# exfinen/zk-toolkit

Hardware: AMD Instinct MI355X
Metric: G1 MSM scalar-muls/sec at 2^20 bases per GPU (BLS12-381) (higher is better)
Workload: dtype u32 limbs (384-bit Montgomery integer)

## Files before the change

zk-toolkit_amd/csrc/curve.h:

```cpp
#pragma once
#include "tower.h"

namespace zkt {

template <class C> struct PrimeOps {
  typedef Fp<C> E;
  ZKT_HD static E zero() { return fp_zero<C>(); }
  ZKT_HD static E one() { return fp_one<C>(); }
  ZKT_HD static E add(const E& a, const E& b) { return fp_add(a, b); }
  ZKT_HD static E sub(const E& a, const E& b) { return fp_sub(a, b); }
  ZKT_HD static E mul(const E& a, const E& b) { return fp_mul(a, b); }
  ZKT_HD static E sqr(const E& a) { return fp_sqr(a); }
  ZKT_HD static E dbl(const E& a) { return fp_dbl(a); }
  ZKT_HD static E sub2(const E& a, const E& b, const E& c) { return fp_sub2(a, b, c); }
  ZKT_HD static E mulsub(const E& a, const E& b, const E& c, const E& d) { return fp_mulsub(a, b, c, d); }
  ZKT_HD static E neg(const E& a) { return fp_neg(a); }
  ZKT_HD static E inv(const E& a) { return fp_inv(a); }
  ZKT_HD static bool is_zero(const E& a) { return fp_is_zero(a); }
  ZKT_HD static bool eq(const E& a, const E& b) { return fp_eq(a, b); }
};
typedef PrimeOps<FqC> FqOps;
typedef PrimeOps<SpC> SpOps;
struct Fq2Ops {
  typedef Fq2 E;
  ZKT_HD static E zero() { return fq2_zero(); }
  ZKT_HD static E one() { return fq2_one(); }
  ZKT_HD static E add(const E& a, const E& b) { return fq2_add(a, b); }
  ZKT_HD static E sub(const E& a, const E& b) { return fq2_sub(a, b); }
  ZKT_HD static E mul(const E& a, const E& b) { return fq2_mul(a, b); }
  ZKT_HD static E sqr(const E& a) { return fq2_sqr(a); }
  ZKT_HD static E dbl(const E& a) { return fq2_dbl(a); }
  ZKT_HD static E sub2(const E& a, const E& b, const E& c) { return fq2_sub2(a, b, c); }
  ZKT_HD static E mulsub(const E& a, const E& b, const E& c, const E& d) { return fq2_mulsub(a, b, c, d); }
  ZKT_HD static E neg(const E& a) { return fq2_neg(a); }
  ZKT_HD static E inv(const E& a) { return fq2_inv(a); }
  ZKT_HD static bool is_zero(const E& a) { return fq2_is_zero(a); }
  ZKT_HD static bool eq(const E& a, const E& b) { return fq2_eq(a, b); }
};

template <class F> struct Aff { typename F::E x, y; bool inf; };
template <class F> struct Jac { typename F::E X, Y, Z; };
template <class F> struct Xyzz { typename F::E X, Y, ZZ, ZZZ; };

template <class F> ZKT_HD Jac<F> jac_inf() { return Jac<F>{F::one(), F::one(), F::zero()}; }
template <class F> ZKT_HD bool jac_is_inf(const Jac<F>& p) { return F::is_zero(p.Z); }
template <class F> ZKT_HD Jac<F> jac_from_aff(const Aff<F>& a) {
  if (a.inf) return jac_inf<F>();
  return Jac<F>{a.x, a.y, F::one()};
}

template <class F> ZKT_HD Jac<F> jac_dbl(const Jac<F>& p) {
  typedef typename F::E E;
  E A = F::sqr(p.X), B = F::sqr(p.Y), C = F::sqr(B);
  E t = F::sqr(F::add(p.X, B));
  E D = F::dbl(F::sub(F::sub(t, A), C));
  E Ee = F::add(F::dbl(A), A);
  E Ff = F::sqr(Ee);
  Jac<F> r;
  r.X = F::sub2(Ff, F::zero(), D);
  E C8 = F::dbl(F::dbl(F::dbl(C)));
  r.Y = F::sub(F::mul(Ee, F::sub(D, r.X)), C8);
  r.Z = F::dbl(F::mul(p.Y, p.Z));
  return r;
}

template <class F> ZKT_HD Jac<F> jac_add_aff(const Jac<F>& p, const Aff<F>& q) {
  typedef typename F::E E;
  if (q.inf) return p;
  if (jac_is_inf(p)) return Jac<F>{q.x, q.y, F::one()};
  E ZZ = F::sqr(p.Z);
  E U2 = F::mul(q.x, ZZ);
  E S2 = F::mul(F::mul(q.y, p.Z), ZZ);
  E H = F::sub(U2, p.X);
  E Rr = F::sub(S2, p.Y);
  if (F::is_zero(H)) {
    if (F::is_zero(Rr)) return jac_dbl(Jac<F>{q.x, q.y, F::one()});
    return jac_inf<F>();
  }
  E HH = F::sqr(H), HHH = F::mul(H, HH), V = F::mul(p.X, HH);
  Jac<F> r;
  r.X = F::sub2(F::sqr(Rr), HHH, V);
  r.Y = F::mulsub(Rr, F::sub(V, r.X), p.Y, HHH);
  r.Z = F::mul(p.Z, H);
  return r;
}

template <class F> ZKT_HD Jac<F> jac_add(const Jac<F>& p, const Jac<F>& q) {
  typedef typename F::E E;
  if (jac_is_inf(q)) return p;
  if (jac_is_inf(p)) return q;
  E Z1Z1 = F::sqr(p.Z), Z2Z2 = F::sqr(q.Z);
  E U1 = F::mul(p.X, Z2Z2), U2 = F::mul(q.X, Z1Z1);
  E S1 = F::mul(F::mul(p.Y, q.Z), Z2Z2), S2 = F::mul(F::mul(q.Y, p.Z), Z1Z1);
  E H = F::sub(U2, U1), Rr = F::sub(S2, S1);
  if (F::is_zero(H)) {
    if (F::is_zero(Rr)) return jac_dbl(p);
    return jac_inf<F>();
  }
  E HH = F::sqr(H), HHH = F::mul(H, HH), V = F::mul(U1, HH);
  Jac<F> r;
  r.X = F::sub2(F::sqr(Rr), HHH, V);
  r.Y = F::mulsub(Rr, F::sub(V, r.X), S1, HHH);
  r.Z = F::mul(F::mul(p.Z, q.Z), H);
  return r;
}

template <class F> ZKT_HD Aff<F> jac_to_aff(const Jac<F>& p) {
  typedef typename F::E E;
  Aff<F> a;
  if (jac_is_inf(p)) { a.x = F::zero(); a.y = F::zero(); a.inf = true; return a; }
  E zi = F::inv(p.Z), zi2 = F::sqr(zi);
  a.x = F::mul(p.X, zi2);
  a.y = F::mul(p.Y, F::mul(zi2, zi));
  a.inf = false;
  return a;
}

template <class F> ZKT_HD Xyzz<F> xyzz_inf() { return Xyzz<F>{F::one(), F::one(), F::zero(), F::zero()}; }
template <class F> ZKT_HD bool xyzz_is_inf(const Xyzz<F>& p) { return F::is_zero(p.ZZ); }
template <class F> ZKT_HD Xyzz<F> xyzz_dbl_aff(const typename F::E& x, const typename F::E& y) {
  typedef typename F::E E;
  if (F::is_zero(y)) return xyzz_inf<F>();
  E U = F::dbl(y), V = F::sqr(U), W = F::mul(U, V), S = F::mul(x, V);
  E xx = F::sqr(x), M = F::add(F::dbl(xx), xx);
  Xyzz<F> r;
  r.X = F::sub2(F::sqr(M), F::zero(), S);
  r.Y = F::mulsub(M, F::sub(S, r.X), W, y);
  r.ZZ = V; r.ZZZ = W;
  return r;
}
template <class F> ZKT_HD Xyzz<F> xyzz_dbl(const Xyzz<F>& p) {
  typedef typename F::E E;
  if (xyzz_is_inf(p) || F::is_zero(p.Y)) return xyzz_inf<F>();
  E U = F::dbl(p.Y), V = F::sqr(U), W = F::mul(U, V), S = F::mul(p.X, V);
  E xx = F::sqr(p.X), M = F::add(F::dbl(xx), xx);
  Xyzz<F> r;
  r.X = F::sub2(F::sqr(M), F::zero(), S);
  r.Y = F::mulsub(M, F::sub(S, r.X), W, p.Y);
  r.ZZ = F::mul(V, p.ZZ); r.ZZZ = F::mul(W, p.ZZZ);
  return r;
}
template <class F> ZKT_HD Xyzz<F> xyzz_add_aff(const Xyzz<F>& p, const typename F::E& x2, const typename F::E& y2) {
  typedef typename F::E E;
  if (xyzz_is_inf(p)) return Xyzz<F>{x2, y2, F::one(), F::one()};
  E U2 = F::mul(x2, p.ZZ), S2 = F::mul(y2, p.ZZZ);
  E Pp = F::sub(U2, p.X), Rr = F::sub(S2, p.Y);
  if (F::is_zero(Pp)) {
    if (F::is_zero(Rr)) return xyzz_dbl_aff<F>(x2, y2);
    return xyzz_inf<F>();
  }
  E PP = F::sqr(Pp), PPP = F::mul(Pp, PP), Qq = F::mul(p.X, PP);
  Xyzz<F> r;
  r.X = F::sub2(F::sqr(Rr), PPP, Qq);
  r.Y = F::mulsub(Rr, F::sub(Qq, r.X), p.Y, PPP);
  r.ZZ = F::mul(p.ZZ, PP); r.ZZZ = F::mul(p.ZZZ, PPP);
  return r;
}
template <class F> ZKT_HD Xyzz<F> xyzz_add(const Xyzz<F>& p, const Xyzz<F>& q) {
  typedef typename F::E E;
  if (xyzz_is_inf(q)) return p;
  if (xyzz_is_inf(p)) return q;
  E U1 = F::mul(p.X, q.ZZ), U2 = F::mul(q.X, p.ZZ);
  E S1 = F::mul(p.Y, q.ZZZ), S2 = F::mul(q.Y, p.ZZZ);
  E Pp = F::sub(U2, U1), Rr = F::sub(S2, S1);
  if (F::is_zero(Pp)) {
    if (F::is_zero(Rr)) return xyzz_dbl(p);
    return xyzz_inf<F>();
  }
  E PP = F::sqr(Pp), PPP = F::mul(Pp, PP), Qq = F::mul(U1, PP);
  Xyzz<F> r;
  r.X = F::sub2(F::sqr(Rr), PPP, Qq);
  r.Y = F::mulsub(Rr, F::sub(Qq, r.X), S1, PPP);
  r.ZZ = F::mul(F::mul(p.ZZ, q.ZZ), PP); r.ZZZ = F::mul(F::mul(p.ZZZ, q.ZZZ), PPP);
  return r;
}
template <class F> ZKT_HD Aff<F> xyzz_to_aff(const Xyzz<F>& p) {
  typedef typename F::E E;
  Aff<F> a;
  if (xyzz_is_inf(p)) { a.x = F::zero(); a.y = F::zero(); a.inf = true; return a; }
  E zi3 = F::inv(p.ZZZ);
  E zi2 = F::sqr(F::mul(zi3, p.ZZ));
  a.x = F::mul(p.X, zi2);
  a.y = F::mul(p.Y, zi3);
  a.inf = false;
  return a;
}
template <class F> ZKT_HD Jac<F> xyzz_to_jac(const Xyzz<F>& p) {
  if (xyzz_is_inf(p)) return jac_inf<F>();
  return Jac<F>{F::mul(p.X, p.ZZ), F::mul(p.Y, p.ZZZ), p.ZZ};
}

static constexpr int SCALAR_MAX_LIMBS = 12;
template <class F> ZKT_HD Jac<F> scalar_mul_aff(const Aff<F>& p, const uint32_t* k, int nlimbs) {
  Jac<F> acc = jac_inf<F>();
  if (p.inf) return acc;
  uint32_t nz[SCALAR_MAX_LIMBS + 1], ng[SCALAR_MAX_LIMBS + 1];
  uint32_t carry = 0;
  for (int w = 0; w <= nlimbs; ++w) {
    const uint32_t cur = w < nlimbs ? k[w] : 0u, nxt = w + 1 < nlimbs ? k[w + 1] : 0u;
    uint32_t znz = 0, zng = 0;
    for (int b = 0; b < 32; ++b) {
      const uint32_t b0 = (cur >> b) & 1, b1 = b < 31 ? (cur >> (b + 1)) & 1 : nxt & 1;
      const uint32_t x0 = b0 ^ carry;
      const uint32_t sum1 = b1 ^ (b0 & carry);
      const uint32_t neg = x0 & sum1;
      znz |= x0 << b; zng |= neg << b;
      carry = (b0 & carry) | (neg);
    }
    nz[w] = znz; ng[w] = zng;
  }
  Aff<F> q = p; q.y = F::neg(p.y);
  bool started = false;
  for (int i = nlimbs * 32; i >= 0; --i) {
    if (started) acc = jac_dbl(acc);
    if ((nz[i >> 5] >> (i & 31)) & 1) { acc = jac_add_aff(acc, ((ng[i >> 5] >> (i & 31)) & 1) ? q : p); started = true; }
  }
  return acc;
}

}
```

zk-toolkit_amd/csrc/fp.h:

```cpp
#pragma once
#include <stdint.h>
#include <hip/hip_runtime.h>
#include "zkt_constants.h"

namespace zkt {

template <class C>
struct Fp {
  typedef uint32_t vec_t __attribute__((ext_vector_type(C::N)));
  vec_t v;
};

ZKT_HD void mac(uint64_t& lo, uint32_t& hi, uint32_t a, uint32_t b) {
#if defined(__HIP_DEVICE_COMPILE__)
  asm("v_mad_u64_u32 %0, vcc, %2, %3, %0\n\tv_addc_co_u32 %1, vcc, 0, %1, vcc" : "+v"(lo), "+v"(hi) : "v"(a), "v"(b) : "vcc");
#else
  uint64_t p = (uint64_t)a * b; lo += p; hi += (lo < p);
#endif
}
ZKT_HD void mac_k(uint64_t& lo, uint32_t& hi, uint32_t a, uint32_t b) {
#if defined(__HIP_DEVICE_COMPILE__)
  asm("v_mad_u64_u32 %0, vcc, %2, %3, %0\n\tv_addc_co_u32 %1, vcc, 0, %1, vcc" : "+v"(lo), "+v"(hi) : "v"(a), "s"(b) : "vcc");
#else
  mac(lo, hi, a, b);
#endif
}
ZKT_HD uint32_t addc(uint32_t a, uint32_t b, uint32_t& c) { unsigned co; uint32_t r = __builtin_addc(a, b, c, &co); c = co; return r; }
ZKT_HD uint32_t subb(uint32_t a, uint32_t b, uint32_t& c) { unsigned co; uint32_t r = __builtin_subc(a, b, c, &co); c = co; return r; }

#define ZKT_FORCE_FRAME() do { alignas(64) volatile uint32_t zkt_frame_anchor_[16]; zkt_frame_anchor_[0] = 0u; } while (0)

template <class C> ZKT_HD Fp<C> fp_zero() { Fp<C> r;
#pragma unroll
  for (int i = 0; i < C::N; ++i) r.v[i] = 0; return r; }
template <class C> ZKT_HD Fp<C> fp_one() { Fp<C> r;
#pragma unroll
  for (int i = 0; i < C::N; ++i) r.v[i] = C::one(i); return r; }
template <class C> ZKT_HD bool fp_is_zero(const Fp<C>& a) {
  if constexpr (C::W == 28) {
    const uint32_t a0 = a.v[0];
    if (!((a0 == C::kp(0, 0)) | (a0 == C::kp(1, 0)) | (a0 == C::kp(2, 0)) | (a0 == C::kp(3, 0)))) return false;
    uint32_t o0 = 0, o1 = 0, o2 = 0, o3 = 0;
#pragma unroll
    for (int i = 0; i < C::N; ++i) { o0 |= a.v[i]; o1 |= a.v[i] ^ C::kp(1, i); o2 |= a.v[i] ^ C::kp(2, i); o3 |= a.v[i] ^ C::kp(3, i); }
    return (o0 == 0) | (o1 == 0) | (o2 == 0) | (o3 == 0);
  } else {
    uint32_t o = 0;
#pragma unroll
    for (int i = 0; i < C::N; ++i) o |= a.v[i];
    return o == 0;
  }
}

template <class C> ZKT_HD void fp_cond_sub(Fp<C>& r, uint32_t top) {
  uint32_t s[C::N]; uint32_t bw = 0;
#pragma unroll
  for (int i = 0; i < C::N; ++i) s[i] = subb(r.v[i], C::mod(i), bw);
  bool keep = (top == 0) && bw;
#pragma unroll
  for (int i = 0; i < C::N; ++i) r.v[i] = keep ? r.v[i] : s[i];
}

template <class C> ZKT_HD Fp<C> fp_lazy_reduce(const uint32_t* v) {
  constexpr uint32_t M = (1u << C::W) - 1;
  Fp<C> r; const uint32_t q = (uint32_t)(((uint64_t)v[C::N - 1] * C::QEST_M) >> 32);
  uint32_t carry = 0;
#pragma unroll
  for (int i = 0; i < C::N; ++i) {
    uint64_t t = (uint64_t)q * C::comp(i) + (uint64_t)(v[i] + carry);
    r.v[i] = (uint32_t)t & M; carry = (uint32_t)(t >> C::W);
  }
  return r;
}

template <class C> ZKT_HD Fp<C> fp_add(const Fp<C>& a, const Fp<C>& b) {
  if constexpr (C::W == 28) {
    uint32_t v[C::N];
#pragma unroll
    for (int i = 0; i < C::N; ++i) v[i] = a.v[i] + b.v[i];
    return fp_lazy_reduce<C>(v);
  } else {
    Fp<C> r; uint32_t c = 0;
#pragma unroll
    for (int i = 0; i < C::N; ++i) r.v[i] = addc(a.v[i], b.v[i], c);
    fp_cond_sub(r, c);
    return r;
  }
}
template <class C> ZKT_HD Fp<C> fp_sub(const Fp<C>& a, const Fp<C>& b) {
  if constexpr (C::W == 28) {
    uint32_t v[C::N];
#pragma unroll
    for (int i = 0; i < C::N; ++i) v[i] = a.v[i] + C::subk(i) - b.v[i];
    return fp_lazy_reduce<C>(v);
  } else {
    Fp<C> r; uint32_t bw = 0;
#pragma unroll
    for (int i = 0; i < C::N; ++i) r.v[i] = subb(a.v[i], b.v[i], bw);
    uint32_t mask = 0u - bw, c = 0;
#pragma unroll
    for (int i = 0; i < C::N; ++i) r.v[i] = addc(r.v[i], C::mod(i) & mask, c);
    return r;
  }
}
template <class C> ZKT_HD Fp<C> fp_neg(const Fp<C>& a) {
  if constexpr (C::W == 28) {
    return fp_sub(fp_zero<C>(), a);
  } else {
    Fp<C> r; uint32_t bw = 0;
#pragma unroll
    for (int i = 0; i < C::N; ++i) r.v[i] = subb(C::mod(i), a.v[i], bw);
    uint32_t mask = fp_is_zero(a) ? 0u : 0xffffffffu;
#pragma unroll
    for (int i = 0; i < C::N; ++i) r.v[i] &= mask;
    return r;
  }
}
template <class C> ZKT_HD bool fp_eq(const Fp<C>& a, const Fp<C>& b) {
  if constexpr (C::W == 28) {
    return fp_is_zero(fp_sub(a, b));
  } else {
    uint32_t o = 0;
#pragma unroll
    for (int i = 0; i < C::N; ++i) o |= a.v[i] ^ b.v[i];
    return o == 0;
  }
}
template <class C> ZKT_HD Fp<C> fp_dbl(const Fp<C>& a) { return fp_add(a, a); }
template <class C> ZKT_HD Fp<C> fp_add3(const Fp<C>& a, const Fp<C>& b, const Fp<C>& c) {
  if constexpr (C::W == 28) {
    uint32_t v[C::N];
#pragma unroll
    for (int i = 0; i < C::N; ++i) v[i] = a.v[i] + b.v[i] + c.v[i];
    return fp_lazy_reduce<C>(v);
  } else return fp_add(fp_add(a, b), c);
}
// ... 74 lines not shown
      lo = (lo >> 32) | ((uint64_t)hi << 32); hi = 0;
    }
    fp_cond_sub(r, (uint32_t)lo);
    return r;
  }
}

template <class C> ZKT_HD Fp<C> fp_sqr_impl(const Fp<C>& a) {
  static_assert(C::W == 28, "lazy-limb fields only");
  constexpr int N = C::N; constexpr uint32_t M = (1u << 28) - 1;
  Fp<C> r; uint32_t m[N], d[N]; uint64_t acc = 0;
#pragma unroll
  for (int i = 0; i < N; ++i) d[i] = a.v[i] << 1;
#pragma unroll
  for (int k = 0; k < 2 * N; ++k) {
#pragma unroll
    for (int i = (k < N ? 0 : k - N + 1); 2 * i < k; ++i) acc = mad64(d[i], a.v[k - i], acc);
    if ((k & 1) == 0) acc = mad64(a.v[k / 2], a.v[k / 2], acc);
    if (k < N) {
#pragma unroll
      for (int j = 0; j < k; ++j) acc = mad64(m[j], C::mod(k - j), acc);
      m[k] = ((uint32_t)acc * C::INV) & M;
      acc = mad64(m[k], C::mod(0), acc);
    } else {
#pragma unroll
      for (int j = k - N + 1; j < N; ++j) acc = mad64(m[j], C::mod(k - j), acc);
      r.v[k - N] = (uint32_t)acc & M;
    }
    acc >>= 28;
  }
  return r;
}

template <class C, bool SUB> ZKT_HD Fp<C> fp_mul2_impl(const Fp<C>& a, const Fp<C>& b, const Fp<C>& c, const Fp<C>& d) {
  static_assert(C::W == 28, "lazy-limb fields only");
  constexpr int N = C::N; constexpr uint32_t M = (1u << 28) - 1;
  Fp<C> r; uint32_t m[N], nd[N]; uint64_t acc = 0;
#pragma unroll
  for (int i = 0; i < N; ++i) nd[i] = SUB ? C::subk(i) - d.v[i] : d.v[i];
#pragma unroll
  for (int k = 0; k < 2 * N; ++k) {
#pragma unroll
    for (int i = (k < N ? 0 : k - N + 1); i <= (k < N ? k : N - 1); ++i) { acc = mad64(a.v[i], b.v[k - i], acc); acc = mad64(c.v[i], nd[k - i], acc); }
    if (k < N) {
#pragma unroll
      for (int j = 0; j < k; ++j) acc = mad64(m[j], C::mod(k - j), acc);
      m[k] = ((uint32_t)acc * C::INV) & M;
      acc = mad64(m[k], C::mod(0), acc);
    } else {
#pragma unroll
      for (int j = k - N + 1; j < N; ++j) acc = mad64(m[j], C::mod(k - j), acc);
      r.v[k - N] = (uint32_t)acc & M;
    }
    acc >>= 28;
  }
  return r;
}

template <class C> ZKT_HD void fp2_mul_kara(const Fp<C>& a0, const Fp<C>& a1, const Fp<C>& b0, const Fp<C>& b1, Fp<C>& re, Fp<C>& im) {
  static_assert(C::W == 28, "lazy-limb fields only");
  constexpr int N = C::N; constexpr uint32_t M = (1u << 28) - 1;
  uint32_t sa[N], sb[N], nd[N], mr[N], mi[N]; uint64_t accr = 0, acci = 0;
#pragma unroll
  for (int i = 0; i < N; ++i) { sa[i] = a0.v[i] + a1.v[i]; sb[i] = b0.v[i] + b1.v[i]; nd[i] = C::subk(i) - b1.v[i]; }
#pragma unroll
  for (int k = 0; k < 2 * N; ++k) {
    uint64_t p0 = 0, p1 = 0;
#pragma unroll
    for (int i = (k < N ? 0 : k - N + 1); i <= (k < N ? k : N - 1); ++i) {
      p0 = mad64(a0.v[i], b0.v[k - i], p0); p1 = mad64(a1.v[i], nd[k - i], p1); acci = mad64(sa[i], sb[k - i], acci);
    }
    accr += p0 + p1; acci += p1 - p0;
    if (k < N) {
#pragma unroll
      for (int j = 0; j < k; ++j) { accr = mad64(mr[j], C::mod(k - j), accr); acci = mad64(mi[j], C::mod(k - j), acci); }
      mr[k] = ((uint32_t)accr * C::INV) & M; mi[k] = ((uint32_t)acci * C::INV) & M;
      accr = mad64(mr[k], C::mod(0), accr); acci = mad64(mi[k], C::mod(0), acci);
    } else {
#pragma unroll
      for (int j = k - N + 1; j < N; ++j) { accr = mad64(mr[j], C::mod(k - j), accr); acci = mad64(mi[j], C::mod(k - j), acci); }
      re.v[k - N] = (uint32_t)accr & M; im.v[k - N] = (uint32_t)acci & M;
    }
    accr >>= 28; acci >>= 28;
  }
}

#if !defined(ZKT_INLINE_MUL)
template <class C> ZKT_FN Fp<C> fp_mul(Fp<C> a, Fp<C> b) { return fp_mul_impl(a, b); }
template <class C> ZKT_FN Fp<C> fp_sqr_fn(Fp<C> a) { return fp_sqr_impl(a); }
#if defined(ZKT_INLINE_MUL2)
template <class C> ZKT_HD Fp<C> fp_mulsub_fn(const Fp<C>& a, const Fp<C>& b, const Fp<C>& c, const Fp<C>& d) { return fp_mul2_impl<C, true>(a, b, c, d); }
template <class C> ZKT_HD Fp<C> fp_muladd_fn(const Fp<C>& a, const Fp<C>& b, const Fp<C>& c, const Fp<C>& d) { return fp_mul2_impl<C, false>(a, b, c, d); }
#else
template <class C> ZKT_FN Fp<C> fp_mulsub_fn(Fp<C> a, Fp<C> b, Fp<C> c, Fp<C> d) { return fp_mul2_impl<C, true>(a, b, c, d); }
template <class C> ZKT_FN Fp<C> fp_muladd_fn(Fp<C> a, Fp<C> b, Fp<C> c, Fp<C> d) { return fp_mul2_impl<C, false>(a, b, c, d); }
#endif
#else
template <class C> ZKT_HD Fp<C> fp_mul(const Fp<C>& a, const Fp<C>& b) { return fp_mul_impl(a, b); }
template <class C> ZKT_HD Fp<C> fp_sqr_fn(const Fp<C>& a) { return fp_sqr_impl(a); }
template <class C> ZKT_HD Fp<C> fp_mulsub_fn(const Fp<C>& a, const Fp<C>& b, const Fp<C>& c, const Fp<C>& d) { return fp_mul2_impl<C, true>(a, b, c, d); }
template <class C> ZKT_HD Fp<C> fp_muladd_fn(const Fp<C>& a, const Fp<C>& b, const Fp<C>& c, const Fp<C>& d) { return fp_mul2_impl<C, false>(a, b, c, d); }
#endif
template <class C> ZKT_HD Fp<C> fp_mulsub(const Fp<C>& a, const Fp<C>& b, const Fp<C>& c, const Fp<C>& d) {
  if constexpr (C::W == 28) return fp_mulsub_fn(a, b, c, d); else return fp_sub(fp_mul(a, b), fp_mul(c, d));
}
template <class C> ZKT_HD Fp<C> fp_muladd(const Fp<C>& a, const Fp<C>& b, const Fp<C>& c, const Fp<C>& d) {
  if constexpr (C::W == 28) return fp_muladd_fn(a, b, c, d); else return fp_add(fp_mul(a, b), fp_mul(c, d));
}

template <class C> ZKT_HD Fp<C> fp_sqr(const Fp<C>& a) {
  if constexpr (C::W == 28) return fp_sqr_fn(a); else return fp_mul(a, a);
}

template <class C> ZKT_HD Fp<C> fp_from_words(const uint32_t* w) {
  Fp<C> x, r2;
#pragma unroll
  for (int i = 0; i < C::N; ++i) r2.v[i] = C::r2(i);
  if constexpr (C::W == 28) {
#pragma unroll
    for (int i = 0; i < C::N; ++i) {
      const int lo = (28 * i) >> 5, sh = (28 * i) & 31;
      uint32_t t = w[lo] >> sh;
      if (sh > 4 && lo + 1 < C::ABI_N) t |= w[lo + 1] << (32 - sh);
      x.v[i] = t & 0x0fffffffu;
    }
  } else {
#pragma unroll
    for (int i = 0; i < C::N; ++i) x.v[i] = w[i];
    x = fp_canon32(x);
  }
  return fp_mul(x, r2);
}
template <class C> ZKT_HD void fp_to_words(const Fp<C>& a, uint32_t* w) {
  Fp<C> one = fp_zero<C>(); one.v[0] = 1;
  Fp<C> x = fp_mul(a, one);
  if constexpr (C::W == 28) {
    uint32_t s[C::N], bw = 0;
#pragma unroll
    for (int i = 0; i < C::N; ++i) { uint32_t t = x.v[i] - C::mod(i) - bw; bw = t >> 31; s[i] = t & 0x0fffffffu; }
#pragma unroll
    for (int i = 0; i < C::N; ++i) s[i] = bw ? x.v[i] : s[i];
#pragma unroll
    for (int j = 0; j < C::ABI_N; ++j) {
      uint32_t t = 0;
#pragma unroll
      for (int i = 0; i < C::N; ++i) {
        const int sft = 28 * i - 32 * j;
        if (sft > -28 && sft < 32) t |= sft >= 0 ? (s[i] << (sft & 31)) : (s[i] >> ((-sft) & 31));
      }
      w[j] = t;
    }
  } else {
#pragma unroll
    for (int i = 0; i < C::N; ++i) w[i] = x.v[i];
  }
}
template <class C> ZKT_HD Fp<C> fp_canon32(Fp<C> x) {
  static_assert(C::W == 32, "canonical 32-bit-limb fields only");
  fp_cond_sub(x, 0); fp_cond_sub(x, 0);
  return x;
}

template <class C> ZKT_HD void bgcd_inverse_classic(uint32_t* io) {
  constexpr int N = C::ABI_N;
  uint32_t u[N + 1], v[N + 1], x1[N + 1], x2[N + 1];
#pragma unroll
  for (int i = 0; i < N; ++i) { u[i] = io[i]; v[i] = C::mod32(i); x1[i] = 0; x2[i] = 0; }
  u[N] = v[N] = x1[N] = x2[N] = 0; x1[0] = 1;
  {
    uint32_t any = 0;
#pragma unroll
    for (int i = 0; i < N; ++i) any |= u[i];
    if (any == 0) return;
  }
  auto is_one = [&](const uint32_t* t) { uint32_t o = t[0] ^ 1u;
#pragma unroll
    for (int i = 1; i <= N; ++i) o |= t[i]; return o == 0; };
  auto shr1 = [&](uint32_t* t) {
#pragma unroll
    for (int i = 0; i < N; ++i) t[i] = (t[i] >> 1) | (t[i + 1] << 31); t[N] >>= 1; };
  auto add_p = [&](uint32_t* t) { uint32_t c = 0;
#pragma unroll
    for (int i = 0; i < N; ++i) t[i] = addc(t[i], C::mod32(i), c); t[N] += c; };
  auto sub = [&](uint32_t* t, const uint32_t* s) { uint32_t b = 0;
#pragma unroll
// ... 177 lines not shown
```

zk-toolkit_amd/csrc/hostcheck.cpp:

```cpp
#include "abi.h"
#include "fq_program.h"
using namespace zkt;

extern "C" {
unsigned long zkt_hostcheck_bgcd_fallbacks() { return bgcd_fallbacks(); }
int zkt_hostcheck_fq_program(uint64_t seed, int steps, const uint32_t* in4, uint32_t* out4) { return fq_program(seed, steps, in4, out4); }
int zkt_hostcheck_fp(int field, int op, const uint32_t* a, const uint32_t* b, uint32_t* o, size_t n) {
  auto run = [&](auto tag) {
    typedef decltype(tag) C;
    for (size_t i = 0; i < n; ++i) {
      if (op == 9 || op == 10) { uint32_t w[C::ABI_N]; for (int j = 0; j < C::ABI_N; ++j) w[j] = a[i * C::ABI_N + j]; if (op == 9) bgcd_inverse_classic<C>(w); else bgcd_inverse<C>(w); for (int j = 0; j < C::ABI_N; ++j) o[i * C::ABI_N + j] = w[j]; continue; }
      Fp<C> x = ld_fp<C>(a + i * C::ABI_N), y = b ? ld_fp<C>(b + i * C::ABI_N) : fp_zero<C>(), r;
      switch (op) {
        case 0: r = fp_add(x, y); break; case 1: r = fp_sub(x, y); break; case 2: r = fp_mul(x, y); break;
        case 3: r = fp_sqr(x); break; case 4: r = fp_neg(x); break; case 6: { uint32_t e[C::ABI_N]; for (int j = 0; j < C::ABI_N; ++j) e[j] = C::pm2(j); r = fp_pow(x, e, C::ABI_N); } break;
        case 7: r = fp_mul(fp_sqr(x), x); break; case 8: r = fp_pow(x, b + i * C::ABI_N, C::ABI_N); break; default: r = fp_inv(x);
      }
      st_fp<C>(o + i * C::ABI_N, r);
    }
  };
  switch (field) { case 0: run(FqC{}); break; case 1: run(FrC{}); break; case 2: run(SpC{}); break; default: run(SnC{}); }
  return 0;
}
int zkt_hostcheck_fq2_mul_lifted(const uint32_t* a, const uint32_t* b, unsigned lifts, uint32_t* o) {
  Fq2 x = ld_fq2(a), y = ld_fq2(b);
  x.c0 = fq_lift(x.c0, (lifts & 3) % 3); x.c1 = fq_lift(x.c1, ((lifts >> 2) & 3) % 3);
  y.c0 = fq_lift(y.c0, ((lifts >> 4) & 3) % 3); y.c1 = fq_lift(y.c1, ((lifts >> 6) & 3) % 3);
  const Fq2 four{fp_mulsub(x.c0, y.c0, x.c1, y.c1), fp_muladd(x.c0, y.c1, x.c1, y.c0)};
  Fq2 three; fp2_mul_kara(x.c0, x.c1, y.c0, y.c1, three.c0, three.c1);
  int bad = 0;
  if (!fq_lazy_ok(three.c0) || !fq_lazy_ok(three.c1)) ++bad;
  if (!fp_eq(four.c0, three.c0) || !fp_eq(four.c1, three.c1)) ++bad;
  st_fq2(o, three);
  return bad;
}
int zkt_hostcheck_tower(int deg, int op, const uint32_t* a, const uint32_t* b, uint32_t* o) {
  if (deg == 2) {
    Fq2 x = ld_fq2(a), y = b ? ld_fq2(b) : fq2_zero(), r;
    switch (op) { case 0: r = fq2_add(x, y); break; case 1: r = fq2_sub(x, y); break; case 2: r = fq2_mul(x, y); break;
      case 3: r = fq2_inv(x); break; case 4: r = fq2_neg(x); break; case 5: r = fq2_mul_xi(x); break; default: r = fq2_sqr(x); }
    st_fq2(o, r);
  } else if (deg == 6) {
    Fq6 x = ld_fq6(a), y = b ? ld_fq6(b) : fq6_zero(), r;
    switch (op) { case 0: r = fq6_add(x, y); break; case 1: r = fq6_sub(x, y); break; case 2: r = fq6_mul(x, y); break;
      case 3: r = fq6_inv(x); break; case 4: r = fq6_neg(x); break; default: r = fq6_mul_v(x); }
    st_fq6(o, r);
  } else {
    Fq12 x = ld_fq12(a), y = b ? ld_fq12(b) : fq12_one(), r;
    switch (op) { case 0: r = fq12_add(x, y); break; case 1: r = fq12_sub(x, y); break; case 2: r = fq12_mul(x, y); break;
      case 3: r = fq12_inv(x); break; case 4: r = fq12_neg(x); break; case 6: r = fq12_sqr(x); break;
      case 7: r = fq12_frob<1>(x); break; case 8: r = fq12_frob<2>(x); break; case 10: r = fq12_cyclotomic_sqr(x); break; default: r = fq12_conj(x); }
    st_fq12(o, r);
  }
  return 0;
}
}
template <class F> static void pt_add(const uint32_t* a, const uint32_t* b, uint32_t* o) {
  Aff<F> p = PtIO<F>::ld(a), q = PtIO<F>::ld(b);
  PtIO<F>::st(o, jac_to_aff(jac_add_aff(jac_from_aff(p), q)));
}
template <class F> static void pt_add_full(const uint32_t* a, const uint32_t* b, uint32_t* o) {
  Aff<F> p = PtIO<F>::ld(a), q = PtIO<F>::ld(b);
  Jac<F> j = jac_add(jac_dbl(jac_from_aff(p)), jac_from_aff(q));
  Aff<F> np = p; if (!np.inf) np.y = F::neg(np.y);
  j = jac_add_aff(j, np);
  Xyzz<F> z = xyzz_inf<F>();
  if (!p.inf) z = xyzz_add_aff(z, p.x, p.y);
  if (!q.inf) z = xyzz_add_aff(z, q.x, q.y);
  Xyzz<F> z2 = xyzz_add(z, xyzz_inf<F>());
  Aff<F> r1 = jac_to_aff(j), r2 = xyzz_to_aff(z2), r3 = jac_to_aff(xyzz_to_jac(z));
  bool same = (r1.inf == r2.inf) && (r1.inf || (F::eq(r1.x, r2.x) && F::eq(r1.y, r2.y)));
  same = same && (r1.inf == r3.inf) && (r1.inf || (F::eq(r1.x, r3.x) && F::eq(r1.y, r3.y)));
  if (!same) { r1.inf = true; }
  PtIO<F>::st(o, r1);
}
template <class F> static void pt_mul(const uint32_t* a, const uint32_t* k, int klimbs, uint32_t* o) {
  PtIO<F>::st(o, jac_to_aff(scalar_mul_aff(PtIO<F>::ld(a), k, klimbs)));
}
extern "C" {
int zkt_hostcheck_group(int grp, int op, const uint32_t* a, const uint32_t* b, int klimbs, uint32_t* o) {
  if (grp == 0) { if (op == 0) pt_add<FqOps>(a, b, o); else if (op == 1) pt_add_full<FqOps>(a, b, o); else pt_mul<FqOps>(a, b, klimbs, o); }
  else if (grp == 1) { if (op == 0) pt_add<Fq2Ops>(a, b, o); else if (op == 1) pt_add_full<Fq2Ops>(a, b, o); else pt_mul<Fq2Ops>(a, b, klimbs, o); }
  else { if (op == 0) pt_add<SpOps>(a, b, o); else if (op == 1) pt_add_full<SpOps>(a, b, o); else pt_mul<SpOps>(a, b, klimbs, o); }
  return 0;
}
int zkt_hostcheck_miller_exact(int which, const uint32_t* g1, const uint32_t* g2, uint32_t* o) {
  Aff<FqOps> p = PtIO<FqOps>::ld(g1); Aff<Fq2Ops> q = PtIO<Fq2Ops>::ld(g2);
  if (p.inf || q.inf) return 2;
  Fq12 r; bool bad = false;
  if (which == 0) r = miller_g1_g2_exact(p.x, p.y, q.x, q.y, bad);
  else if (which == 1) r = miller_g2_g1_exact(q.x, q.y, p.x, p.y);
  else r = fq12_mul(miller_g1_g2_exact(p.x, p.y, q.x, q.y, bad), fq12_inv(miller_g2_g1_exact(q.x, q.y, p.x, p.y)));
  if (bad) return 2;
  st_fq12(o, r);
  return 0;
}
int zkt_hostcheck_tate(const uint32_t* g1, const uint32_t* g2, uint32_t* o) {
  Aff<FqOps> p = PtIO<FqOps>::ld(g1); Aff<Fq2Ops> q = PtIO<Fq2Ops>::ld(g2);
  if (p.inf || q.inf) return 2;
  Fq12 f; bool in_g1 = false, bad;
  const int route = tate_short(p.x, p.y, q.x, q.y, f);
  if (route == TATE_ROUTE_SHORT) { st_fq12(o, f); return 0; }
  if (route == TATE_ROUTE_LONG) {
    f = miller_g1_g2(p.x, p.y, q.x, q.y, in_g1);
    if (in_g1) { st_fq12(o, final_exponentiation(f)); return 50; }
  }
  f = miller_g1_g2_exact(p.x, p.y, q.x, q.y, bad);
  if (bad) return 2;
  if (fq12_is_zero(f)) { for (int k = 0; k < 144; ++k) o[k] = 0; return 100; }
  st_fq12(o, final_exponentiation(f));
  return 100;
}
int zkt_hostcheck_short_loop_guards(const uint32_t* g1, const uint32_t* g2) {
  Aff<FqOps> p = PtIO<FqOps>::ld(g1); Aff<Fq2Ops> q = PtIO<Fq2Ops>::ld(g2);
  if (p.inf || q.inf) return -1;
  bool ok; (void)miller_g1_g2_short(p.x, p.y, q.x, q.y, ok);
// ... 33 lines not shown
```

zk-toolkit_amd/csrc/zkt_msm.hip:

```cpp
#include <cstdlib>
#include "abi.h"
#include "zkt_internal.h"

namespace zkt {

#ifndef ZKT_SIDE_PRIO
#define ZKT_SIDE_PRIO __builtin_amdgcn_s_setprio(3)
#endif
template <class F> struct Coord;
template <class C> struct Coord<PrimeOps<C>> {
  static constexpr int CW = C::N;
  __device__ static Fp<C> ld(const uint32_t* p) { return ld_raw<C>(p); }
  __device__ static void st(uint32_t* p, const Fp<C>& a) { st_raw<C>(p, a); }
};
template <> struct Coord<Fq2Ops> {
  static constexpr int CW = 2 * FqC::N;
  __device__ static Fq2 ld(const uint32_t* p) { Fq2 r; r.c0 = ld_raw<FqC>(p); r.c1 = ld_raw<FqC>(p + FqC::N); return r; }
  __device__ static void st(uint32_t* p, const Fq2& a) { st_raw<FqC>(p, a.c0); st_raw<FqC>(p + FqC::N, a.c1); }
};
template <class F> __device__ inline Xyzz<F> ld_xy(const uint32_t* p) {
  constexpr int CW = Coord<F>::CW; Xyzz<F> r;
  r.X = Coord<F>::ld(p); r.Y = Coord<F>::ld(p + CW); r.ZZ = Coord<F>::ld(p + 2 * CW); r.ZZZ = Coord<F>::ld(p + 3 * CW); return r;
}
template <class F> __device__ inline void st_xy(uint32_t* p, const Xyzz<F>& a) {
// ... 350 lines not shown
}

static constexpr uint32_t CHUNK = 128;
static constexpr int SIZE_BINS = CHUNK + 1;
__device__ inline uint32_t ntasks_of(uint32_t c, uint32_t chunk) { return c <= chunk ? 1u : (c + chunk - 1) / chunk; }
__device__ inline uint32_t task_size_of(uint32_t c, uint32_t nt) { return (c + nt - 1) / nt; }
static __global__ void __launch_bounds__(256) k_task_count(const uint32_t* __restrict__ counts, size_t m, uint32_t chunk, uint32_t* __restrict__ ntask, uint32_t* __restrict__ hist) {
  ZKT_SIDE_PRIO;
  __shared__ uint32_t h[SIZE_BINS];
  for (int i = threadIdx.x; i < SIZE_BINS; i += 256) h[i] = 0;
  __syncthreads();
  size_t i = (size_t)blockIdx.x * 256 + threadIdx.x;
  if (i < m) {
    uint32_t c = counts[i], nt = ntasks_of(c, chunk);
    ntask[i] = nt;
    atomicAdd(&h[CHUNK - task_size_of(c, nt)], nt);
  }
  __syncthreads();
  for (int k = threadIdx.x; k < SIZE_BINS; k += 256) if (h[k]) atomicAdd(&hist[k], h[k]);
}
static constexpr uint32_t HOT_NT = 512, HOT_CAP = 64, HOT_FAN = 64;
static __global__ void __launch_bounds__(256) k_task_scatter(const uint32_t* __restrict__ counts, size_t m, uint32_t chunk, const uint32_t* __restrict__ size_hist,
                                                      uint32_t* __restrict__ bincur, uint2* __restrict__ order, uint32_t* __restrict__ hot) {
  ZKT_SIDE_PRIO;
  __shared__ uint32_t h[SIZE_BINS], base[SIZE_BINS], binoff[SIZE_BINS + 1], scan[256];
  __shared__ uint32_t hot_n, hot_b[256], hot_pos[256], hot_nt[256];
  for (int i = threadIdx.x; i < SIZE_BINS; i += 256) h[i] = 0;
  if (threadIdx.x == 0) hot_n = 0;
  {
    static_assert(SIZE_BINS <= 256, "one histogram bin per thread");
    uint32_t v = threadIdx.x < SIZE_BINS ? size_hist[threadIdx.x] : 0, tot;
    uint32_t ex = block_excl_scan_256(v, scan, tot);
    if (threadIdx.x < SIZE_BINS) binoff[threadIdx.x] = ex;
  }
  __syncthreads();
  size_t i = (size_t)blockIdx.x * 256 + threadIdx.x;
  uint32_t bin = 0, rank = 0, nt = 1;
  if (i < m) { uint32_t c = counts[i]; nt = ntasks_of(c, chunk); bin = CHUNK - task_size_of(c, nt); rank = atomicAdd(&h[bin], nt); }
  __syncthreads();
  for (int k = threadIdx.x; k < SIZE_BINS; k += 256) if (h[k]) base[k] = binoff[k] + atomicAdd(&bincur[k], h[k]);
  __syncthreads();
  if (i < m) {
    const uint32_t pos = base[bin] + rank;
    if (nt <= 16) { for (uint32_t k = 0; k < nt; ++k) order[pos + k] = make_uint2((uint32_t)i, k); }
    else { const uint32_t slot = atomicAdd(&hot_n, 1u); hot_b[slot] = (uint32_t)i; hot_pos[slot] = pos; hot_nt[slot] = nt; }
    if (nt > HOT_NT) { const uint32_t g = atomicAdd(&hot[0], 1u); if (g < HOT_CAP) hot[1 + g] = (uint32_t)i; }
  }
  __syncthreads();
  for (uint32_t hb = 0; hb < hot_n; ++hb) {
    const uint32_t b = hot_b[hb], pos = hot_pos[hb], cnt = hot_nt[hb];
    for (uint32_t k = threadIdx.x; k < cnt; k += 256) order[pos + k] = make_uint2(b, k);
  }
}

#ifndef ZKT_ACC_ATTR
#define ZKT_ACC_ATTR
#endif
template <class F>
__global__ void __launch_bounds__(64) ZKT_ACC_ATTR k_accumulate(const uint32_t* __restrict__ table, const uint32_t* __restrict__ entries,
                                                   const uint32_t* __restrict__ offsets, const uint2* __restrict__ order,
                                                   const uint32_t* __restrict__ task_off, size_t nbuckets,
                                                   uint32_t* __restrict__ sums, uint32_t* __restrict__ partial) {
  size_t t = (size_t)blockIdx.x * 64 + threadIdx.x;
  if (t >= task_off[nbuckets]) return;
  const uint2 tk = order[t];
  const size_t b = tk.x;
  const uint32_t t0 = task_off[b], nt = task_off[b + 1] - t0;
  const uint32_t off = offsets[b], cnt = offsets[b + 1] - off;
  uint32_t beg = off, end = off + cnt;
  if (nt != 1) {
    const uint32_t q = cnt / nt, r = cnt - q * nt;
    beg = off + tk.y * q + (tk.y < r ? tk.y : r); end = beg + q + (tk.y < r ? 1u : 0u);
  }
  constexpr int CW = Coord<F>::CW, XYW = 4 * CW;
  Xyzz<F> acc = xyzz_inf<F>();
  typedef typename F::E E;
  uint32_t ent = beg < end ? entries[beg] : 0, ent_next = beg + 1 < end ? entries[beg + 1] : 0;
  const uint32_t* p = table + (size_t)(ent & 0x7fffffffu) * (2 * CW);
#ifndef ZKT_ACC_PREFETCH_MAX_CW
#define ZKT_ACC_PREFETCH_MAX_CW 16
#endif
  if constexpr (CW <= ZKT_ACC_PREFETCH_MAX_CW) {
    E nx = Coord<F>::ld(p), ny = Coord<F>::ld(p + CW);
    for (uint32_t e = beg; e < end; ++e) {
      E x = nx, y = ny;
      const bool negate = ent >> 31;
      if (e + 1 < end) {
        ent = ent_next;
        ent_next = e + 2 < end ? entries[e + 2] : 0;
        p = table + (size_t)(ent & 0x7fffffffu) * (2 * CW);
        nx = Coord<F>::ld(p); ny = Coord<F>::ld(p + CW);
      }
      if (negate) y = F::neg(y);
      acc = xyzz_add_aff<F>(acc, x, y);
    }
  } else {
    for (uint32_t e = beg; e < end; ++e) {
      E x = Coord<F>::ld(p), y = Coord<F>::ld(p + CW);
      const bool negate = ent >> 31;
      ent = ent_next;
      ent_next = e + 2 < end ? entries[e + 2] : 0;
      p = table + (size_t)(ent & 0x7fffffffu) * (2 * CW);
      if (negate) y = F::neg(y);
      acc = xyzz_add_aff<F>(acc, x, y);
    }
  }
  st_xy<F>(nt == 1 ? sums + b * XYW : partial + (size_t)(t0 + tk.y) * XYW, acc);
}

}
#include "msm_reduce_coop.h"
namespace zkt {

template <class F>
__global__ void __launch_bounds__(64) k_join_windows(const uint32_t* __restrict__ win_jac, int nwin, int c, uint32_t* __restrict__ out_jac, uint32_t* __restrict__ out_abi) {
  ZKT_SIDE_PRIO;
  constexpr int CW = Coord<F>::CW, XYW = 4 * CW, JW = 3 * CW;
  __shared__ uint32_t lds[16 * JW];
  const int t = threadIdx.x;
  auto ldj = [](const uint32_t* p) { return Jac<F>{Coord<F>::ld(p), Coord<F>::ld(p + CW), Coord<F>::ld(p + 2 * CW)}; };
  auto stj = [](uint32_t* p, const Jac<F>& a) { Coord<F>::st(p, a.X); Coord<F>::st(p + CW, a.Y); Coord<F>::st(p + 2 * CW, a.Z); };
  Jac<F> v = jac_inf<F>();
  if (t < nwin) {
    v = ldj(win_jac + (size_t)t * XYW);
    for (int d = 0; d < c * t; ++d) v = jac_dbl(v);
  }
  for (int d = 16; d >= 1; d >>= 1) {
    if (t >= d && t < 2 * d) stj(lds + (t - d) * JW, v);
    __syncthreads();
    if (t < d) v = jac_add(v, ldj(lds + t * JW));
    __syncthreads();
  }
  if (t == 0) {
    stj(out_jac, v);
    if (out_abi) PtIO<F>::st(out_abi, jac_to_aff(v));
  }
}

namespace {
struct MsmWs {
  uint32_t *zero_begin, *counts, *cursor, *size_hist, *size_off, *size_cur, *hot, *zero_end;
  uint32_t *offsets, *entries, *slot, *sums, *colsum, *rowsum, *clsA, *clsB, *win_jac, *scan_tmp, *ntask, *task_off, *partial, *hot_part;
  uint32_t *tilehist, *tileoff, *blkoff, *subhist, *part_scan; uint2* rec;
  uint2* order; size_t max_tasks;
};
MsmWs carve(const MsmPlan& P, void* workspace) {
  const size_t B = P.nbuckets, XYW = 4 * (size_t)coord_words(P.grp);
  uint8_t* ws = (uint8_t*)workspace;
  MsmWs w;
  w.zero_begin = (uint32_t*)ws;
  w.counts = (uint32_t*)ws; ws += (B + 1) * 4;
  w.cursor = (uint32_t*)ws; ws += (B + 1) * 4;
  w.size_hist = (uint32_t*)ws; ws += (SIZE_BINS + 1) * 4;
  w.size_off = (uint32_t*)ws; ws += (SIZE_BINS + 1) * 4;
  w.size_cur = (uint32_t*)ws; ws += (SIZE_BINS + 1) * 4;
  w.hot = (uint32_t*)ws; ws += (HOT_CAP + 1) * 4;
  w.zero_end = (uint32_t*)ws;
  w.offsets = (uint32_t*)ws; ws += (B + 1) * 4;
  ws = (uint8_t*)(((uintptr_t)ws + 255) & ~(uintptr_t)255);
  w.entries = (uint32_t*)ws; ws += (size_t)P.nwin * P.n * 4;
  ws = (uint8_t*)(((uintptr_t)ws + 255) & ~(uintptr_t)255);
  w.slot = (uint32_t*)ws; ws += (size_t)P.nwin * P.n * 4;
  ws = (uint8_t*)(((uintptr_t)ws + 255) & ~(uintptr_t)255);
  w.sums = (uint32_t*)ws; ws += B * XYW * 4;
  const size_t nw = P.direct ? (size_t)P.nwin : 1;
  w.colsum = (uint32_t*)ws; ws += nw * 1024 * XYW * 4;
  w.rowsum = (uint32_t*)ws; ws += nw * 1024 * XYW * 4;
  w.clsA = (uint32_t*)ws; ws += nw * 32 * WB_SPLIT * XYW * 4;
  w.clsB = (uint32_t*)ws; ws += nw * 32 * WB_SPLIT * XYW * 4;
  w.win_jac = (uint32_t*)ws; ws += nw * XYW * 4;
  w.scan_tmp = (uint32_t*)ws; ws += 1024 * 4;
  w.ntask = (uint32_t*)ws; ws += (B + 1) * 4;
  w.task_off = (uint32_t*)ws; ws += (B + 1) * 4;
  w.max_tasks = B + (size_t)P.nwin * P.n / P.chunk + 1;
  ws = (uint8_t*)(((uintptr_t)ws + 255) & ~(uintptr_t)255);
  w.order = (uint2*)ws; ws += w.max_tasks * 8;
  w.partial = (uint32_t*)ws; ws += w.max_tasks * XYW * 4;
// ... 172 lines not shown
```

Before: 417.9 million.

## Add paired chained Montgomery muls and streamlined XYZZ affine accumulation in bucket kernel

Adds a column-wise chained Montgomery multiply, square and mul2 built on inline v_mad_u64_u32, plus paired variants that interleave two independent products, using different carry outputs, for instruction-level parallelism. A new in-place XYZZ affine accumulate uses these pairs, screens for exceptional cases with a cheap low-limb maybe-zero test before the full zero check, and the bucket accumulation loop seeds the accumulator from the first point so it can skip the infinity check. The paired chain path is only taken when ZKT_CHAIN_MUL and ZKT_INLINE_MUL are defined; otherwise the pairs fall back to two ordinary muls. The pairing raises register pressure, and the inline asm constrains scheduling.

```diff
diff --git a/zk-toolkit_amd/csrc/curve.h b/zk-toolkit_amd/csrc/curve.h
--- a/zk-toolkit_amd/csrc/curve.h
+++ b/zk-toolkit_amd/csrc/curve.h
@@ -14,9 +14,12 @@
   ZKT_HD static E dbl(const E& a) { return fp_dbl(a); }
   ZKT_HD static E sub2(const E& a, const E& b, const E& c) { return fp_sub2(a, b, c); }
   ZKT_HD static E mulsub(const E& a, const E& b, const E& c, const E& d) { return fp_mulsub(a, b, c, d); }
+  ZKT_HD static void mul_pair(const E& a, const E& b, const E& c, const E& d, E& ab, E& cd) { fp_mul_pair(a, b, c, d, ab, cd); }
+  ZKT_HD static void sqr_pair(const E& a, const E& c, E& aa, E& cc) { fp_sqr_pair(a, c, aa, cc); }
   ZKT_HD static E neg(const E& a) { return fp_neg(a); }
   ZKT_HD static E inv(const E& a) { return fp_inv(a); }
   ZKT_HD static bool is_zero(const E& a) { return fp_is_zero(a); }
+  ZKT_HD static bool maybe_zero(const E& a) { return fp_maybe_zero(a); }
   ZKT_HD static bool eq(const E& a, const E& b) { return fp_eq(a, b); }
 };
 typedef PrimeOps<FqC> FqOps;
@@ -156,6 +159,27 @@
   r.ZZ = F::mul(p.ZZ, PP); r.ZZZ = F::mul(p.ZZZ, PPP);
   return r;
 }
+template <class F> ZKT_HD void xyzz_acc_aff(Xyzz<F>& p, bool& inf, const typename F::E& x2, const typename F::E& y2) {
+  typedef typename F::E E;
+  E U2, S2; F::mul_pair(x2, p.ZZ, y2, p.ZZZ, U2, S2);
+  const E Pp = F::sub(U2, p.X), Rr = F::sub(S2, p.Y);
+  bool exc = inf | F::maybe_zero(Pp);
+  if (__builtin_expect(exc, 0)) exc = inf | F::is_zero(Pp);
+  if (__builtin_expect(exc, 0)) {
+    if (inf) p = Xyzz<F>{x2, y2, F::one(), F::one()};
+    else if (F::is_zero(Rr)) p = xyzz_dbl_aff<F>(x2, y2);
+    else p = xyzz_inf<F>();
+    inf = xyzz_is_inf(p);
+    return;
+  }
+  E PP, RR; F::sqr_pair(Pp, Rr, PP, RR);
+  E PPP, Qq; F::mul_pair(Pp, PP, p.X, PP, PPP, Qq);
+  Xyzz<F> r;
+  r.X = F::sub2(RR, PPP, Qq);
+  r.Y = F::mulsub(Rr, F::sub(Qq, r.X), p.Y, PPP);
+  F::mul_pair(p.ZZ, PP, p.ZZZ, PPP, r.ZZ, r.ZZZ);
+  p = r;
+}
 template <class F> ZKT_HD Xyzz<F> xyzz_add(const Xyzz<F>& p, const Xyzz<F>& q) {
   typedef typename F::E E;
   if (xyzz_is_inf(q)) return p;
diff --git a/zk-toolkit_amd/csrc/fp.h b/zk-toolkit_amd/csrc/fp.h
--- a/zk-toolkit_amd/csrc/fp.h
+++ b/zk-toolkit_amd/csrc/fp.h
@@ -52,6 +52,15 @@
   }
 }
 
+template <class C> ZKT_HD bool fp_maybe_zero(const Fp<C>& a) {
+  if constexpr (C::W == 28) {
+    const uint32_t a0 = a.v[0];
+    return (a0 == C::kp(0, 0)) | (a0 == C::kp(1, 0)) | (a0 == C::kp(2, 0)) | (a0 == C::kp(3, 0));
+  } else {
+    return a.v[0] == 0;
+  }
+}
+
 template <class C> ZKT_HD void fp_cond_sub(Fp<C>& r, uint32_t top) {
   uint32_t s[C::N]; uint32_t bw = 0;
 #pragma unroll
@@ -292,6 +301,116 @@
       re.v[k - N] = (uint32_t)accr & M; im.v[k - N] = (uint32_t)acci & M;
     }
     accr >>= 28; acci >>= 28;
+  }
+}
+
+template <int S = 0> ZKT_HD uint64_t mad_vv(uint32_t a, uint32_t b, uint64_t c) {
+#if defined(__HIP_DEVICE_COMPILE__)
+  if constexpr (S) asm("v_mad_u64_u32 %0, vcc, %1, %2, %0" : "+&v"(c) : "v"(a), "v"(b) : "vcc");
+  else { uint64_t co; asm("v_mad_u64_u32 %0, %1, %2, %3, %0" : "+&v"(c), "=s"(co) : "v"(a), "v"(b)); }
+  return c;
+#else
+  return (uint64_t)a * b + c;
+#endif
+}
+template <int S = 0> ZKT_HD uint64_t mad_vs(uint32_t a, uint32_t b, uint64_t c) {
+#if defined(__HIP_DEVICE_COMPILE__)
+  if constexpr (S) asm("v_mad_u64_u32 %0, vcc, %1, %2, %0" : "+&v"(c) : "v"(a), "s"(b) : "vcc");
+  else { uint64_t co; asm("v_mad_u64_u32 %0, %1, %2, %3, %0" : "+&v"(c), "=s"(co) : "v"(a), "s"(b)); }
+  return c;
+#else
+  return (uint64_t)a * b + c;
+#endif
+}
+template <int S = 0> ZKT_HD uint64_t mul_vv(uint32_t a, uint32_t b) {
+#if defined(__HIP_DEVICE_COMPILE__)
+  uint64_t r;
+  if constexpr (S) asm("v_mad_u64_u32 %0, vcc, %1, %2, 0" : "=&v"(r) : "v"(a), "v"(b) : "vcc");
+  else { uint64_t co; asm("v_mad_u64_u32 %0, %1, %2, %3, 0" : "=&v"(r), "=s"(co) : "v"(a), "v"(b)); }
+  return r;
+#else
+  return (uint64_t)a * b;
+#endif
+}
+template <class C, int S = 0> ZKT_HD uint64_t chain_mul_col(uint64_t acc, const Fp<C>& a, const Fp<C>& b, int k) {
+  constexpr int N = C::N;
+#pragma unroll
+  for (int i = (k < N ? 0 : k - N + 1); i <= (k < N ? k : N - 1); ++i) acc = (k == 0) ? mul_vv<S>(a.v[i], b.v[k - i]) : mad_vv<S>(a.v[i], b.v[k - i], acc);
+  return acc;
+}
+template <class C, int S = 0> ZKT_HD uint64_t chain_sqr_col(uint64_t acc, const Fp<C>& a, const uint32_t* d, int k) {
+  constexpr int N = C::N;
+#pragma unroll
+  for (int i = (k < N ? 0 : k - N + 1); 2 * i < k; ++i) acc = mad_vv<S>(d[i], a.v[k - i], acc);
+  if ((k & 1) == 0) acc = (k == 0) ? mul_vv<S>(a.v[0], a.v[0]) : mad_vv<S>(a.v[k / 2], a.v[k / 2], acc);
+  return acc;
+}
+template <class C, int S = 0> ZKT_HD uint64_t chain_mul2_col(uint64_t acc, const Fp<C>& a, const Fp<C>& b, const Fp<C>& c, const uint32_t* nd, int k) {
+  constexpr int N = C::N;
+#pragma unroll
+  for (int i = (k < N ? 0 : k - N + 1); i <= (k < N ? k : N - 1); ++i) {
+    acc = (k == 0) ? mul_vv<S>(a.v[i], b.v[k - i]) : mad_vv<S>(a.v[i], b.v[k - i], acc);
+    acc = mad_vv<S>(c.v[i], nd[k - i], acc);
+  }
+  return acc;
+}
+template <class C, int S = 0> ZKT_HD uint64_t chain_red_col(uint64_t acc, uint32_t* m, Fp<C>& r, int k) {
+  constexpr int N = C::N; constexpr uint32_t M = (1u << 28) - 1;
+  if (k < N) {
+#pragma unroll
+    for (int j = 0; j < k; ++j) acc = mad_vs<S>(m[j], C::mod(k - j), acc);
+    m[k] = ((uint32_t)acc * C::INV) & M;
+    acc = mad_vs<S>(m[k], C::mod(0), acc);
+  } else {
+#pragma unroll
+    for (int j = k - N + 1; j < N; ++j) acc = mad_vs<S>(m[j], C::mod(k - j), acc);
+    r.v[k - N] = (uint32_t)acc & M;
+  }
+  return acc >> 28;
+}
+template <class C> ZKT_HD Fp<C> fp_mul_chain(const Fp<C>& a, const Fp<C>& b) {
+  static_assert(C::W == 28, "lazy-limb fields only");
+  Fp<C> r; uint32_t m[C::N]; uint64_t acc = 0;
+#pragma unroll
+  for (int k = 0; k < 2 * C::N; ++k) acc = chain_red_col<C>(chain_mul_col<C>(acc, a, b, k), m, r, k);
+  return r;
+}
+template <class C> ZKT_HD Fp<C> fp_sqr_chain(const Fp<C>& a) {
+  static_assert(C::W == 28, "lazy-limb fields only");
+  Fp<C> r; uint32_t m[C::N], d[C::N]; uint64_t acc = 0;
+#pragma unroll
+  for (int i = 0; i < C::N; ++i) d[i] = a.v[i] << 1;
+#pragma unroll
+  for (int k = 0; k < 2 * C::N; ++k) acc = chain_red_col<C>(chain_sqr_col<C>(acc, a, d, k), m, r, k);
+  return r;
+}
+template <class C, bool SUB> ZKT_HD Fp<C> fp_mul2_chain(const Fp<C>& a, const Fp<C>& b, const Fp<C>& c, const Fp<C>& d) {
+  static_assert(C::W == 28, "lazy-limb fields only");
+  Fp<C> r; uint32_t m[C::N], nd[C::N]; uint64_t acc = 0;
+#pragma unroll
+  for (int i = 0; i < C::N; ++i) nd[i] = SUB ? C::subk(i) - d.v[i] : d.v[i];
+#pragma unroll
+  for (int k = 0; k < 2 * C::N; ++k) acc = chain_red_col<C>(chain_mul2_col<C>(acc, a, b, c, nd, k), m, r, k);
+  return r;
+}
+template <class C> ZKT_HD void fp_mul_pair_chain(const Fp<C>& a, const Fp<C>& b, const Fp<C>& c, const Fp<C>& d, Fp<C>& ab, Fp<C>& cd) {
+  static_assert(C::W == 28, "lazy-limb fields only");
+  uint32_t m0[C::N], m1[C::N]; uint64_t acc0 = 0, acc1 = 0;
+#pragma unroll
+  for (int k = 0; k < 2 * C::N; ++k) {
+    acc0 = chain_mul_col<C, 0>(acc0, a, b, k); acc1 = chain_mul_col<C, 1>(acc1, c, d, k);
+    acc0 = chain_red_col<C, 0>(acc0, m0, ab, k); acc1 = chain_red_col<C, 1>(acc1, m1, cd, k);
+  }
+}
+template <class C> ZKT_HD void fp_sqr_pair_chain(const Fp<C>& a, const Fp<C>& c, Fp<C>& aa, Fp<C>& cc) {
+  static_assert(C::W == 28, "lazy-limb fields only");
+  uint32_t m0[C::N], m1[C::N], da[C::N], dc[C::N]; uint64_t acc0 = 0, acc1 = 0;
+#pragma unroll
+  for (int i = 0; i < C::N; ++i) { da[i] = a.v[i] << 1; dc[i] = c.v[i] << 1; }
+#pragma unroll
+  for (int k = 0; k < 2 * C::N; ++k) {
+    acc0 = chain_sqr_col<C, 0>(acc0, a, da, k); acc1 = chain_sqr_col<C, 1>(acc1, c, dc, k);
+    acc0 = chain_red_col<C, 0>(acc0, m0, aa, k); acc1 = chain_red_col<C, 1>(acc1, m1, cc, k);
   }
 }
 
@@ -305,12 +424,29 @@
 template <class C> ZKT_FN Fp<C> fp_mulsub_fn(Fp<C> a, Fp<C> b, Fp<C> c, Fp<C> d) { return fp_mul2_impl<C, true>(a, b, c, d); }
 template <class C> ZKT_FN Fp<C> fp_muladd_fn(Fp<C> a, Fp<C> b, Fp<C> c, Fp<C> d) { return fp_mul2_impl<C, false>(a, b, c, d); }
 #endif
+#elif defined(ZKT_CHAIN_MUL)
+template <class C> ZKT_HD Fp<C> fp_mul(const Fp<C>& a, const Fp<C>& b) { if constexpr (C::W == 28) return fp_mul_chain(a, b); else return fp_mul_impl(a, b); }
+template <class C> ZKT_HD Fp<C> fp_sqr_fn(const Fp<C>& a) { return fp_sqr_chain(a); }
+template <class C> ZKT_HD Fp<C> fp_mulsub_fn(const Fp<C>& a, const Fp<C>& b, const Fp<C>& c, const Fp<C>& d) { return fp_mul2_chain<C, true>(a, b, c, d); }
+template <class C> ZKT_HD Fp<C> fp_muladd_fn(const Fp<C>& a, const Fp<C>& b, const Fp<C>& c, const Fp<C>& d) { return fp_mul2_chain<C, false>(a, b, c, d); }
 #else
 template <class C> ZKT_HD Fp<C> fp_mul(const Fp<C>& a, const Fp<C>& b) { return fp_mul_impl(a, b); }
 template <class C> ZKT_HD Fp<C> fp_sqr_fn(const Fp<C>& a) { return fp_sqr_impl(a); }
 template <class C> ZKT_HD Fp<C> fp_mulsub_fn(const Fp<C>& a, const Fp<C>& b, const Fp<C>& c, const Fp<C>& d) { return fp_mul2_impl<C, true>(a, b, c, d); }
 template <class C> ZKT_HD Fp<C> fp_muladd_fn(const Fp<C>& a, const Fp<C>& b, const Fp<C>& c, const Fp<C>& d) { return fp_mul2_impl<C, false>(a, b, c, d); }
 #endif
+template <class C> ZKT_HD void fp_mul_pair(const Fp<C>& a, const Fp<C>& b, const Fp<C>& c, const Fp<C>& d, Fp<C>& ab, Fp<C>& cd) {
+#if defined(ZKT_CHAIN_MUL) && defined(ZKT_INLINE_MUL)
+  if constexpr (C::W == 28) { fp_mul_pair_chain(a, b, c, d, ab, cd); return; }
+#endif
+  ab = fp_mul(a, b); cd = fp_mul(c, d);
+}
+template <class C> ZKT_HD void fp_sqr_pair(const Fp<C>& a, const Fp<C>& c, Fp<C>& aa, Fp<C>& cc) {
+#if defined(ZKT_CHAIN_MUL) && defined(ZKT_INLINE_MUL)
+  if constexpr (C::W == 28) { fp_sqr_pair_chain(a, c, aa, cc); return; }
+#endif
+  aa = fp_sqr(a); cc = fp_sqr(c);
+}
 template <class C> ZKT_HD Fp<C> fp_mulsub(const Fp<C>& a, const Fp<C>& b, const Fp<C>& c, const Fp<C>& d) {
   if constexpr (C::W == 28) return fp_mulsub_fn(a, b, c, d); else return fp_sub(fp_mul(a, b), fp_mul(c, d));
 }
diff --git a/zk-toolkit_amd/csrc/hostcheck.cpp b/zk-toolkit_amd/csrc/hostcheck.cpp
--- a/zk-toolkit_amd/csrc/hostcheck.cpp
+++ b/zk-toolkit_amd/csrc/hostcheck.cpp
@@ -32,6 +32,29 @@
   if (!fq_lazy_ok(three.c0) || !fq_lazy_ok(three.c1)) ++bad;
   if (!fp_eq(four.c0, three.c0) || !fp_eq(four.c1, three.c1)) ++bad;
   st_fq2(o, three);
+  return bad;
+}
+int zkt_hostcheck_fq_chain(int op, const uint32_t* a, const uint32_t* b, const uint32_t* c, const uint32_t* d, uint32_t* o, uint32_t* o2, size_t n) {
+  constexpr int N = FqC::N;
+  auto ld = [](const uint32_t* w) { Fp<FqC> x; for (int j = 0; j < N; ++j) x.v[j] = w[j]; return x; };
+  auto st = [](uint32_t* w, const Fp<FqC>& x) { for (int j = 0; j < N; ++j) w[j] = x.v[j]; };
+  auto same = [](const Fp<FqC>& x, const Fp<FqC>& y) { for (int j = 0; j < N; ++j) if (x.v[j] != y.v[j]) return false; return true; };
+  int bad = 0;
+  for (size_t i = 0; i < n; ++i) {
+    const Fp<FqC> x = ld(a + i * N), y = ld(b + i * N), z = ld(c + i * N), w = ld(d + i * N);
+    Fp<FqC> r, r2, want, want2;
+    switch (op) {
+      case 0: r = fp_mul_chain(x, y); want = fp_mul_impl(x, y); break;
+      case 1: r = fp_sqr_chain(x); want = fp_sqr_impl(x); break;
+      case 2: r = fp_mul2_chain<FqC, true>(x, y, z, w); want = fp_mul2_impl<FqC, true>(x, y, z, w); break;
+      case 3: r = fp_mul2_chain<FqC, false>(x, y, z, w); want = fp_mul2_impl<FqC, false>(x, y, z, w); break;
+      case 4: fp_mul_pair_chain(x, y, z, w, r, r2); want = fp_mul_impl(x, y); want2 = fp_mul_impl(z, w); break;
+      default: fp_sqr_pair_chain(x, z, r, r2); want = fp_sqr_impl(x); want2 = fp_sqr_impl(z); break;
+    }
+    st(o + i * N, r);
+    if (!same(r, want)) ++bad;
+    if (op >= 4) { st(o2 + i * N, r2); if (!same(r2, want2)) ++bad; }
+  }
   return bad;
 }
 int zkt_hostcheck_tower(int deg, int op, const uint32_t* a, const uint32_t* b, uint32_t* o) {
diff --git a/zk-toolkit_amd/csrc/zkt_msm.hip b/zk-toolkit_amd/csrc/zkt_msm.hip
--- a/zk-toolkit_amd/csrc/zkt_msm.hip
+++ b/zk-toolkit_amd/csrc/zkt_msm.hip
@@ -456,8 +456,8 @@
 #endif
   if constexpr (CW <= ZKT_ACC_PREFETCH_MAX_CW) {
     E nx = Coord<F>::ld(p), ny = Coord<F>::ld(p + CW);
-    for (uint32_t e = beg; e < end; ++e) {
-      E x = nx, y = ny;
+    auto take = [&](uint32_t e, E& x, E& y) {
+      x = nx; y = ny;
       const bool negate = ent >> 31;
       if (e + 1 < end) {
         ent = ent_next;
@@ -466,7 +466,12 @@
         nx = Coord<F>::ld(p); ny = Coord<F>::ld(p + CW);
       }
       if (negate) y = F::neg(y);
-      acc = xyzz_add_aff<F>(acc, x, y);
+    };
+    if (beg < end) {
+      E x, y; take(beg, x, y);
+      acc = Xyzz<F>{x, y, F::one(), F::one()};
+      bool inf = false;
+      for (uint32_t e = beg + 1; e < end; ++e) { take(e, x, y); xyzz_acc_aff<F>(acc, inf, x, y); }
     }
   } else {
     for (uint32_t e = beg; e < end; ++e) {
```

Result: faster. 425.4 million (median of 6 runs) (+1.8%).
